# myroslavlisniak/lsm_storage_engine

Hardware: AMD Instinct MI355X
Metric: GiB/s device-resident batched record checksum; % of HBM3E read BW (higher is better)
Workload: dtype u8; 1 GPU; config3: 67108864 mixed-length records per GPU (64 B-64 KiB, Zipf s=1.5, packed, unaligned; 97.0 GiB), device-resident; records_per_gpu=67108864, payload_bytes_per_gpu=104143148313, parallelism=record-sharded x1, no data-path collective, checksum=CRC-32/ISO-HDLC (crc::crc32::checksum_ieee)

## Files before the change

lsm_storage_engine_amd/csrc/lsmck_crc32.hip:

```cpp
#include <hip/hip_runtime.h>
#include <stdint.h>
#ifdef LSMCK_WAVE_DIAG
#include <stdio.h>
#include <stdlib.h>

#include <vector>
#endif

#include "lsmck_device.h"
#include "lsmck_splan.h"

namespace lsmck {

typedef unsigned int u32x4 __attribute__((ext_vector_type(4)));

#define LDS_TABLE_BYTES 131072u
#define LDS_SHIFT_OFF 131072u
#define LDS_SHIFT_BYTES 12288u
#define LDS_COLS_OFF (LDS_SHIFT_OFF + LDS_SHIFT_BYTES)
#define LDS_COLS_BYTES 8192u
#define LDS_KHI_OFF (LDS_COLS_OFF + LDS_COLS_BYTES)
#define LDS_KHI_BYTES 2048u
#define LDS_KLO_OFF (LDS_KHI_OFF + LDS_KHI_BYTES)
#define LDS_KMID_OFF (LDS_KLO_OFF + 2048u)
#define LDS_TINIT_OFF (LDS_KMID_OFF + 512u)
#define LDS_SCRATCH_OFF (LDS_TINIT_OFF + 544u)
#define WAVE_SCRATCH_BYTES 256u
#define LDS_SMAP_OFF LDS_SCRATCH_OFF
#define LDS_SMAP_BYTES 4096u
__device__ __forceinline__ uint32_t gf2_mulmod(uint32_t a, uint32_t b) {
  uint32_t p = 0;
#pragma unroll
  for (int i = 0; i < 32; ++i) {
    uint32_t m = (uint32_t)((int32_t)(a << i) >> 31);
    p ^= b & m;
    b = (b >> 1) ^ (0xEDB88320u & (0u - (b & 1u)));
  }
  return p;
}

__host__ __device__ __forceinline__ uint32_t segs_of(uint32_t len) { return (len >> 7) + ((len & 127u) != 0u); }

typedef __attribute__((address_space(3))) const uint32_t lds_u32_t;
typedef __attribute__((address_space(3))) const u32x4 lds_u32x4_t;
__device__ __forceinline__ uint32_t lds_ld(const unsigned char* smem, uint32_t a) {
  (void)smem;
  return *(lds_u32_t*)(size_t)a;
}
__device__ __forceinline__ u32x4 lds_ld128(uint32_t a) { return *(lds_u32x4_t*)(size_t)a; }

__device__ __forceinline__ void build_lds_tables(unsigned char* smem, const CrcParams& P) {
  const uint32_t* __restrict__ master = P.master;
  uint32_t* s32 = (uint32_t*)smem;
  for (uint32_t i = threadIdx.x; i < LDS_TABLE_BYTES / 4; i += blockDim.x) {
    uint32_t t = ((i >> 14) << 1) | ((i >> 5) & 1u);
    uint32_t e = (i >> 6) & 255u;
    s32[i] = master[t * 256u + e];
  }
  for (uint32_t i = threadIdx.x; i < LDS_SHIFT_BYTES / 4; i += blockDim.x) s32[LDS_SHIFT_OFF / 4 + i] = master[1024u + i];
  for (uint32_t i = threadIdx.x; i < LDS_KHI_BYTES / 4; i += blockDim.x) s32[LDS_KHI_OFF / 4 + i] = P.khi[i];
  for (uint32_t i = threadIdx.x; i < 512u; i += blockDim.x) s32[LDS_KLO_OFF / 4 + i] = P.kseg[i];
  for (uint32_t i = threadIdx.x; i < 128u; i += blockDim.x) s32[LDS_KMID_OFF / 4 + i] = P.kseg[512u * i];
  for (uint32_t i = threadIdx.x; i < 130u; i += blockDim.x) s32[LDS_TINIT_OFF / 4 + i] = P.tinit[i];
}

template <int M>
__device__ __forceinline__ uint32_t shift_bytes32(const unsigned char* smem, uint32_t s) {
  constexpr uint32_t base = LDS_SHIFT_OFF + (M - 1) * 4096u;
  return lds_ld(smem, base + ((s & 0xFFu) << 2)) ^ lds_ld(smem, base + 1024u + (((s >> 8) & 0xFFu) << 2)) ^
         lds_ld(smem, base + 2048u + (((s >> 16) & 0xFFu) << 2)) ^ lds_ld(smem, base + 3072u + ((s >> 24) << 2));
}


__device__ __forceinline__ uint32_t crc_word(const unsigned char* smem, uint32_t s, uint32_t w, uint32_t lo,
                                             uint32_t hi) {
  uint32_t x = s ^ w;
  uint32_t a0 = __builtin_amdgcn_perm(x, hi, 0x0c020400u);
  uint32_t a1 = __builtin_amdgcn_perm(x, hi, 0x0c020500u);
  uint32_t a2 = __builtin_amdgcn_perm(x, lo, 0x0c0c0600u);
  uint32_t a3 = __builtin_amdgcn_perm(x, lo, 0x0c0c0700u);
  return lds_ld(smem, a0 + 128u) ^ lds_ld(smem, a1) ^ lds_ld(smem, a2 + 128u) ^ lds_ld(smem, a3);
}

__device__ __forceinline__ uint32_t crc_step_x(const unsigned char* smem, uint32_t x, uint32_t w_next, uint32_t lo,
                                               uint32_t hi) {
  uint32_t a0 = __builtin_amdgcn_perm(x, hi, 0x0c020400u);
  uint32_t a1 = __builtin_amdgcn_perm(x, hi, 0x0c020500u);
  uint32_t a2 = __builtin_amdgcn_perm(x, lo, 0x0c0c0600u);
  uint32_t a3 = __builtin_amdgcn_perm(x, lo, 0x0c0c0700u);
  const uint32_t l2 = lds_ld(smem, a2 + 128u), l3 = lds_ld(smem, a3);
  const uint32_t t = __builtin_amdgcn_bitop3_b32(l2, l3, w_next, 0x96);
  return __builtin_amdgcn_bitop3_b32(lds_ld(smem, a0 + 128u), lds_ld(smem, a1), t, 0x96);
}

__device__ __forceinline__ void crc_step_x2(uint32_t& c0, uint32_t& c1, uint32_t x0, uint32_t n0, uint32_t x1,
                                            uint32_t n1, uint32_t lo, uint32_t hi) {
  const uint32_t a00 = __builtin_amdgcn_perm(x0, hi, 0x0c020400u), a01 = __builtin_amdgcn_perm(x0, hi, 0x0c020500u);
  const uint32_t a02 = __builtin_amdgcn_perm(x0, lo, 0x0c0c0600u), a03 = __builtin_amdgcn_perm(x0, lo, 0x0c0c0700u);
  const uint32_t a10 = __builtin_amdgcn_perm(x1, hi, 0x0c020400u), a11 = __builtin_amdgcn_perm(x1, hi, 0x0c020500u);
  const uint32_t a12 = __builtin_amdgcn_perm(x1, lo, 0x0c0c0600u), a13 = __builtin_amdgcn_perm(x1, lo, 0x0c0c0700u);
  const uint32_t l02 = lds_ld(nullptr, a02 + 128u), l03 = lds_ld(nullptr, a03);
  const uint32_t l00 = lds_ld(nullptr, a00 + 128u), l01 = lds_ld(nullptr, a01);
  const uint32_t l12 = lds_ld(nullptr, a12 + 128u), l13 = lds_ld(nullptr, a13);
  const uint32_t l10 = lds_ld(nullptr, a10 + 128u), l11 = lds_ld(nullptr, a11);
  c0 = __builtin_amdgcn_bitop3_b32(l00, l01, __builtin_amdgcn_bitop3_b32(l02, l03, n0, 0x96), 0x96);
  c1 = __builtin_amdgcn_bitop3_b32(l10, l11, __builtin_amdgcn_bitop3_b32(l12, l13, n1, 0x96), 0x96);
}

__device__ __forceinline__ uint32_t ld32(const unsigned char* p) { return *(const uint32_t*)p; }
__device__ __forceinline__ u32x4 ld128(const unsigned char* p) { return *(const u32x4*)p; }

template <typename T>
__device__ __forceinline__ void keep_live(const T& x) {
  asm volatile("" ::"v"(x));
}

struct SegInfo {
  uint32_t rec;
  uint32_t q;
  uint32_t k;
  uint64_t rec_off;
  uint32_t rec_len;
  bool valid;
};

struct SegLoad {
  uint32_t d[33];
  uint32_t rec, k;
  uint32_t fl;
};
#define FL_SH(f) ((f) & 3u)
#define FL_BST(f) (((f) >> 2) & 0xFFu)
#define FL_VALID 0x400u
#define FL_FIRST 0x800u
#define FL_M(f) (((f) >> 12) & 0x3Fu)

template <bool FAST, int ABLATE = 0>
__device__ __forceinline__ void seg_issue(const CrcParams& P, const SegInfo& si, SegLoad& L) {
  const uint64_t E = si.rec_off + si.rec_len - 128ull * si.k;
  const uint32_t seglen = (si.q == 0) ? si.rec_len - 128u * si.k : 128u;
  const uint32_t lead = 128u - seglen;
  L.rec = si.rec;
  L.k = si.k;
  const uint32_t flv = (si.valid ? FL_VALID : 0u) | (si.q == 0 ? FL_FIRST : 0u);
  L.fl = flv;
  const unsigned char* s0 = P.base + (E - 128);
  if (FAST) {
#pragma unroll
    for (int g = 0; g < 8; ++g) {
      u32x4 v = ld128(s0 + 16 * g);
      L.d[4 * g + 0] = v.x;
      L.d[4 * g + 1] = v.y;
      L.d[4 * g + 2] = v.z;
      L.d[4 * g + 3] = v.w;
    }
    keep_live(s0);
    L.d[32] = 0;
    return;
  }
  const uint32_t sh = (uint32_t)((uintptr_t)s0 & 3);
  const unsigned char* p = s0 - sh;
  const uint32_t bstart = sh + lead;
  const bool empty = lead >= 128u;
  const uintptr_t pa = (uintptr_t)p;
  const uintptr_t pg = (pa + bstart) & ~(uintptr_t)4095;
  const bool cross = !empty & (pg > pa);
  const uint32_t m = cross ? (uint32_t)(pg - pa) >> 2 : 0u;
  L.fl = flv | sh | (bstart << 2) | (m << 12);
  const unsigned char* w = empty ? (const unsigned char*)P.zero : p + 4u * m;
#pragma unroll
  for (int g = 0; g < 8; ++g) {
    u32x4 v = ld128(w + 16 * g);
    L.d[4 * g + 0] = v.x;
    L.d[4 * g + 1] = v.y;
    L.d[4 * g + 2] = v.z;
    L.d[4 * g + 3] = v.w;
  }
  L.d[32] = ld32(w + ((sh != 0u && m == 0u) ? 128 : 124));
  keep_live(w);
}

template <bool FAST, int CHAINS, int ABLATE = 0, bool PERCOL = false, bool RAW = false>
// ... 653 lines not shown
                                  lds_ld(nullptr, (((v >> 10) & 0x3C0u) | bA) + 4096u), 0x96);
  u = __builtin_amdgcn_bitop3_b32(u, lds_ld(nullptr, (((v >> 14) & 0x3C0u) | bA) + 5120u),
                                  lds_ld(nullptr, (((v >> 18) & 0x3C0u) | bA) + 6144u), 0x96);
  u ^= lds_ld(nullptr, (((v >> 22) & 0x3C0u) | bA) + 7168u);
  uint32_t y = __builtin_amdgcn_bitop3_b32(lds_ld(nullptr, ((u << 2) & 0x3Cu) | bB),
                                           lds_ld(nullptr, (((u >> 2) & 0x3Cu) | bB) + 256u),
                                           lds_ld(nullptr, (((u >> 6) & 0x3Cu) | bB) + 512u), 0x96);
  y = __builtin_amdgcn_bitop3_b32(y, lds_ld(nullptr, (((u >> 10) & 0x3Cu) | bB) + 768u),
                                  lds_ld(nullptr, (((u >> 14) & 0x3Cu) | bB) + 1024u), 0x96);
  y = __builtin_amdgcn_bitop3_b32(y, lds_ld(nullptr, (((u >> 18) & 0x3Cu) | bB) + 1280u),
                                  lds_ld(nullptr, (((u >> 22) & 0x3Cu) | bB) + 1536u), 0x96);
  return y ^ lds_ld(nullptr, (((u >> 26) & 0x3Cu) | bB) + 1792u);
}

__device__ __forceinline__ uint32_t stream_capture(const unsigned char* smem, uint32_t cx, uint32_t u, uint32_t t,
                                                   uint32_t lo) {
  const uint32_t b0 = t == 1u ? lo : (t == 2u ? lo + 128u : (lo | 0x10000u));
  const uint32_t b1 = t == 2u ? lo : lo + 128u;
  const uint32_t l0 = lds_ld(smem, __builtin_amdgcn_perm(cx, b0, 0x0c020400u));
  const uint32_t l1 = lds_ld(smem, __builtin_amdgcn_perm(cx, b1, 0x0c020500u));
  const uint32_t l2 = lds_ld(smem, __builtin_amdgcn_perm(cx, lo, 0x0c020600u));
  return ((cx ^ u) >> (t << 3)) ^ (t >= 1u ? l0 : 0u) ^ (t >= 2u ? l1 : 0u) ^ (t >= 3u ? l2 : 0u);
}


__device__ __forceinline__ void stream_cut(const CrcParams& P, uint32_t w, uint32_t S, uint32_t W) {
  const uint64_t n = P.nrec;
  if (w == S) {
    P.scuts[w] = n;
    return;
  }
  const uint64_t o0 = P.off[0], dend = P.off[n - 1] + P.len[n - 1];
  const uint64_t target = o0 + (uint64_t)((double)(dend - o0) * splan::fraction(w, S, W));
  uint64_t a = 0, b = n;
  while (a < b) {
    const uint64_t m = (a + b) >> 1;
    if (P.off[m] < target) a = m + 1; else b = m;
  }
  P.scuts[w] = a;
}

template <bool VEC>
__global__ __launch_bounds__(256) void stream_check(CrcParams P, uint32_t S, uint32_t W) {
  const uint64_t n = P.nrec;
  const uint32_t gt = blockIdx.x * 256u + threadIdx.x;
  if (gt == 0u) P.sflag[1] = 0u;
  if (gt <= S) stream_cut(P, gt, S, W);
  const uint64_t i0 = (uint64_t)gt * 4u;
  uint64_t o[5];
  uint32_t l[5];
  if (VEC && i0 + 4u <= n) {
    const u32x4 a = *(const u32x4*)(P.off + i0), b = *(const u32x4*)(P.off + i0 + 2u);
    const u32x4 c = *(const u32x4*)(P.len + i0);
    o[0] = ((uint64_t)a.y << 32) | a.x;
    o[1] = ((uint64_t)a.w << 32) | a.z;
    o[2] = ((uint64_t)b.y << 32) | b.x;
    o[3] = ((uint64_t)b.w << 32) | b.z;
    l[0] = c.x; l[1] = c.y; l[2] = c.z; l[3] = c.w;
  } else {
#pragma unroll
    for (int j = 0; j < 4; ++j) {
      const uint64_t i = i0 + j < n ? i0 + j : n - 1u;
      o[j] = P.off[i];
      l[j] = P.len[i];
    }
  }
  o[4] = ((uint64_t)(uint32_t)__shfl_down((int)(uint32_t)(o[0] >> 32), 1) << 32) | (uint32_t)__shfl_down((int)(uint32_t)o[0], 1);
  l[4] = (uint32_t)__shfl_down((int)l[0], 1);
  if ((threadIdx.x & 63u) == 63u && i0 + 4u < n) {
    o[4] = P.off[i0 + 4u];
    l[4] = P.len[i0 + 4u];
  }
  bool bad = i0 == 0 && n > 0 && l[0] == 0u;
#pragma unroll
  for (int j = 0; j < 4; ++j) {
    const uint64_t e = o[j] + l[j];
    bad = bad || (i0 + j + 1u < n && (o[j + 1] < e || o[j + 1] - e > STREAM_MAX_GAP || (l[j + 1] == 0u && o[j + 1] != e)));
  }
  if (bad) *P.sflag = 0u;
}

__global__ __launch_bounds__(256) void stream_cuts(CrcParams P, uint32_t S, uint32_t W) {
  const uint32_t w = blockIdx.x * blockDim.x + threadIdx.x;
  if (w == 0u) P.sflag[1] = 0u;
  if (w > S || !*P.sflag) return;
  stream_cut(P, w, S, W);
}

template <int ABLATE>
__device__ __forceinline__ void stream_issue(const CrcParams& P, int64_t tb, uintptr_t end4, uint32_t lane,
                                             uint32_t (&u)[32], uint32_t c0 = 0u) {
  const uintptr_t t0 = (uintptr_t)P.base + (uintptr_t)tb;
  const uint64_t span = end4 - t0;
  const __amdgpu_buffer_rsrc_t r = __builtin_amdgcn_make_buffer_rsrc(
      const_cast<unsigned char*>(P.base + tb), (short)0, (int)(span < 0x7FFFFFFFull ? span : 0x7FFFFFFFull), 0x00020000);
  const uint32_t vo = lane >= c0 ? lane * 128u : 0x80000000u;
  if (ABLATE == 2 || ABLATE == 4 || ABLATE == 10 || ABLATE == 11) {
#pragma unroll
    for (int j = 0; j < 32; ++j) u[j] = (uint32_t)tb * 0x9E3779B1u + lane + j;
    return;
  }
#pragma unroll
  for (int g = 0; g < 8; ++g) {
    auto v = __builtin_amdgcn_raw_buffer_load_b128(r, vo + 16u * g, 0, 0);
    u[4 * g + 0] = v[0];
    u[4 * g + 1] = v[1];
    u[4 * g + 2] = v[2];
    u[4 * g + 3] = v[3];
  }
  keep_live(vo);
}

__device__ __forceinline__ uint32_t stream_short(const CrcParams& P, const unsigned char* smem, int64_t tb, int32_t re,
                                                 uint32_t L, bool on, uint32_t jmin, uint32_t lo, uint32_t hi) {
  const __amdgpu_buffer_rsrc_t r = __builtin_amdgcn_make_buffer_rsrc(
      const_cast<unsigned char*>(P.base + (tb - 256)), (short)0, 8192 + 256, 0x00020000);
  const uint32_t e = (uint32_t)(re + 256);
  const uint32_t s = e - L;
  const uint32_t w0 = e - 64u;
  const uint32_t sh = (uint32_t)(((uintptr_t)P.base + (uintptr_t)(tb - 256) + w0) & 3u);
  const uint32_t p4 = w0 - sh;
  uint32_t d[17];
#pragma unroll
  for (int i = 0; i < 17; ++i) {
    const uint32_t a = p4 + 4u * i;
    const bool hit = on && a + 4u > s && a < e;
    d[i] = __builtin_amdgcn_raw_buffer_load_b32(r, hit ? a : 0x80000000u, 0, 0);
  }
  const uint32_t lead = 64u - L;
  uint32_t c = 0;
#pragma unroll
  for (int j = 0; j < 16; ++j) {
    if ((uint32_t)j < jmin) continue;
    uint32_t w = __builtin_amdgcn_alignbyte(d[j + 1], d[j], sh);
    const uint32_t b = 4u * j;
    w = (b + 4u <= lead) ? 0u : (b >= lead ? w : w & (0xFFFFFFFFu << ((lead - b) << 3)));
    c = crc_word(smem, c, w, lo, hi);
  }
  return ~(c ^ lds_ld(smem, LDS_TINIT_OFF + (L << 2)));
}

__device__ __forceinline__ uint32_t horner(uint32_t v, uint32_t d) {
#ifdef LSMCK_HORNER_COLS
  return walk_mulcol(v, d);
#else
  return nib_mul<LDS_NIBA_OFF, LDS_NIBB_OFF>(v, d);
#endif
}

__device__ __forceinline__ uint32_t finish_mul(uint32_t v, uint32_t m) { return stream_mulcol(v, LDS_XMC_OFF(m)); }

#ifdef LSMCK_WAVE_DIAG
#define LSMCK_WAVE_DIAG_MAX 8192u
__device__ uint64_t g_wave_diag[LSMCK_WAVE_DIAG_MAX][4];
#define WAVE_DIAG(...) __VA_ARGS__
#else
#define WAVE_DIAG(...)
#endif

template <int ABLATE = 0>
__global__ __launch_bounds__(1024) void crc32_stream_kernel(CrcParams P) {
  if (!*P.sflag) return;
  WAVE_DIAG(const uint64_t diag_t0 = wall_clock64(); uint32_t diag_ev = 0; uint32_t diag_no = 0;)
  WAVE_DIAG(auto diag_out = [&] {
    const uint32_t w = (blockIdx.x * blockDim.x + threadIdx.x) >> 6;
    if ((threadIdx.x & 63u) == 0u && w < LSMCK_WAVE_DIAG_MAX) {
      g_wave_diag[w][0] = diag_t0;
      g_wave_diag[w][1] = wall_clock64();
      g_wave_diag[w][2] = ((uint64_t)diag_ev << 32) | diag_no;
      g_wave_diag[w][3] = (uint64_t)__builtin_amdgcn_s_getreg((31 << 11) | 4) |
                          ((uint64_t)__builtin_amdgcn_s_getreg((31 << 11) | 20) << 32);
    }
  };)
  extern __shared__ __attribute__((aligned(16))) unsigned char smem[];
  build_lds_tables(smem, P);
  __syncthreads();
#ifdef LSMCK_HORNER_COLS
  build_walk_cols(P);
#else
  build_nib<LDS_NIBA_OFF, LDS_NIBB_OFF>([&](uint32_t e) { return P.kseg[e]; });
#endif
  if (threadIdx.x >= 128u && threadIdx.x < 192u) {
    const uint32_t f = threadIdx.x - 128u;
    uint32_t K = 0x80000000u;
    for (uint32_t i = 0; i < f; ++i) K = (K >> 8) ^ lds_ld(smem, 256u * (K & 0xFFu));
    const uint32_t base = LDS_XMC_OFF(f);
    for (uint32_t i = 0; i < 32u; ++i) {
      *(__attribute__((address_space(3))) uint32_t*)(size_t)(base + 4u * i) = K;
      K = (K >> 1) ^ (0xEDB88320u & (0u - (K & 1u)));
    }
  }
  const uint32_t lane = threadIdx.x & 63u;
  const uint32_t smap = LDS_SMAP_OFF + (threadIdx.x >> 6) * 256u;
  *(__attribute__((address_space(3))) uint32_t*)(size_t)(smap + 4u * lane) = 0u;
  __syncthreads();
  const uint32_t lo = (lane & 31u) * 4u, hi = lo | 0x10000u;
  const uint32_t wave = __builtin_amdgcn_readfirstlane((blockIdx.x * blockDim.x + threadIdx.x) >> 6);
  const uint64_t n = P.nrec;
  const int64_t a0 = (int64_t)((((uintptr_t)P.base + P.off[0]) & ~(uintptr_t)127) - (uintptr_t)P.base);
  typedef __attribute__((address_space(4))) const CrcParams kargs_t;
  kargs_t* ka = (kargs_t*)__builtin_amdgcn_kernarg_segment_ptr();
  for (uint32_t slice = wave;;) {
  asm volatile("" : "+s"(ka));
  const uint32_t nslice = ka->nslice, nwaves = ka->nwaves;
  if (slice >= nslice) break;
  auto uni64 = [](uint64_t v) -> uint64_t {
    return ((uint64_t)(uint32_t)__builtin_amdgcn_readfirstlane((int)(uint32_t)(v >> 32)) << 32) |
           (uint32_t)__builtin_amdgcn_readfirstlane((int)(uint32_t)v);
  };
  const uint64_t r_lo = uni64(ka->scuts[slice]), r_hi = uni64(ka->scuts[slice + 1]);
  if (nslice > nwaves) {
    uint32_t tk = 0;
    if (lane == 0u) tk = atomicAdd(ka->sflag + 1, 1u);
    slice = nwaves + (uint32_t)__builtin_amdgcn_readfirstlane((int)tk);
  } else {
    slice = nslice;
  }
  if (r_lo >= r_hi) continue;
  const uint64_t o_lo = uni64(P.off[r_lo]), e_hi = uni64(P.off[r_hi - 1] + P.len[r_hi - 1]);
  const uint64_t t_first = (uint64_t)((int64_t)o_lo - a0) >> 13;
  const uint64_t t_last = (uint64_t)((int64_t)e_hi - a0) >> 13;
  const uint32_t c_first = (uint32_t)((uint64_t)((int64_t)o_lo - a0) >> 7) & 63u;
  const uintptr_t end4 = ((uintptr_t)P.base + e_hi + 3u) & ~(uintptr_t)3;
  const uint64_t ntile = t_last >= t_first ? t_last - t_first + 1u : 0u;
  auto tbase = [&](uint64_t t) -> int64_t { return a0 + (int64_t)(t << 13); };

  uint64_t Wo;
  uint32_t Wl;
  auto win_load = [&](uint64_t b) {
    const uint64_t i = b + lane;
    const uint64_t ic = i < n ? i : n - 1u;
    Wo = P.off[ic];
    Wl = P.len[ic];
  };
  uint64_t bt = r_lo;
  uint32_t carry = 0;
  win_load(bt);
  uint32_t qv = 0;
  uint64_t qb = r_lo & ~63ull;
  uint32_t qs = (uint32_t)(r_lo & 63u), qf = qs;
  auto qstore = [&](uint32_t v, bool on, uint32_t* out) {
    const __amdgpu_buffer_rsrc_t r =
        __builtin_amdgcn_make_buffer_rsrc((void*)(out + qb), (short)0, 256, 0x00020000);
    if (on && (ABLATE != 6 || v == 0x9E3779B1u)) __builtin_amdgcn_raw_buffer_store_b32(v, r, lane << 2, 0, 0);
  };
  auto qpush = [&](uint32_t v, uint32_t cnt) {
    const uint32_t src = (lane - qf) & 63u;
    const uint32_t val = (uint32_t)__builtin_amdgcn_ds_bpermute((int)(src << 2), (int)v);
    const uint32_t end = qf + cnt;
    qv = (lane >= qf && lane < end) ? val : qv;
    if (end >= 64u) {
      qstore(qv, lane >= qs, P.out);
      qb += 64u;
      qs = 0u;
      qf = end - 64u;
      qv = lane < qf ? val : qv;
    } else {
      qf = end;
    }
  };

  auto bulk = [&](const uint32_t (&U)[32]) {
    if constexpr (ABLATE == 11 || ABLATE == 12) {
      uint32_t y0 = U[0] ^ (lane == 0u ? carry : 0u), y1 = U[8], y2 = U[16], y3 = U[24];
#pragma unroll
      for (int k = 0; k < 8; ++k) {
        y0 = crc_step_x(smem, y0, k + 1 < 8 ? U[k + 1] : 0u, lo, hi);
        y1 = crc_step_x(smem, y1, k + 1 < 8 ? U[9 + k] : 0u, lo, hi);
        y2 = crc_step_x(smem, y2, k + 1 < 8 ? U[17 + k] : 0u, lo, hi);
        y3 = crc_step_x(smem, y3, k + 1 < 8 ? U[25 + k] : 0u, lo, hi);
      }
      uint32_t dy = 63u - lane;
      asm volatile("" : "+v"(dy));
      const uint32_t XY = wave_prefix_xor(horner(shift_bytes32<2>(smem, y0 ^ y1) ^ y2 ^ y3, dy));
      carry = (uint32_t)__builtin_amdgcn_readlane((int)XY, 63);
      return;
    }
    uint32_t z0 = U[0] ^ (lane == 0u ? carry : 0u), z1 = U[16];
#pragma unroll
    for (int k = 0; k < 16; ++k) {
      z0 = crc_step_x(smem, z0, k + 1 < 16 ? U[k + 1] : 0u, lo, hi);
      z1 = crc_step_x(smem, z1, k + 1 < 16 ? U[17 + k] : 0u, lo, hi);
    }
    uint32_t dz = 63u - lane;
    asm volatile("" : "+v"(dz));
    const uint32_t XZ = wave_prefix_xor(horner(shift_bytes32<2>(smem, z0) ^ z1, dz));
    carry = (uint32_t)__builtin_amdgcn_readlane((int)XZ, 63);
  };

  auto process = [&](const uint32_t (&U)[32], uint64_t t, auto&& issue_next) {
    const int64_t tb = tbase(t);
    if constexpr (ABLATE == 9 || ABLATE == 10 || ABLATE == 11) {
      issue_next();
      __builtin_amdgcn_sched_barrier(0);
      bulk(U);
      return;
    }
    bool zf = false;
    if constexpr (ABLATE == 0 || ABLATE >= 6) {
      const uint32_t so_lo = (uint32_t)__builtin_amdgcn_readfirstlane((int)(uint32_t)Wo);
      const uint32_t so_hi = (uint32_t)__builtin_amdgcn_readfirstlane((int)(uint32_t)(Wo >> 32));
      const uint32_t sl = (uint32_t)__builtin_amdgcn_readfirstlane((int)Wl);
      const int64_t s0 = (int64_t)(((uint64_t)so_hi << 32) | so_lo) - tb;
      zf = bt >= r_hi || (s0 + (int64_t)sl >= 8192 && (s0 < 0 || sl < STREAM_LONG));
    }
    uint32_t Kw = 0;
    bool shorts = false;
    uint64_t wb = bt;
    uint32_t nwin = 0;
    uint32_t cntw = 0;
    int32_t re = 8191, rs = 8191;
    bool lng = false, sin = false;
    const uint64_t bt0 = bt;
    bool z = zf;
    if (!zf) {
      for (;;) {
        const int64_t e64 = (int64_t)(Wo + Wl) - tb, s64 = (int64_t)Wo - tb;
        const bool inr = wb + lane < r_hi;
        const bool ends = inr && e64 < 8192;
        cntw = (uint32_t)__builtin_popcountll(__ballot(ends));
        lng = Wl >= STREAM_LONG;
        sin = inr && s64 >= 0 && s64 < 8192;
        re = (int32_t)(ends ? e64 : 8191);
        rs = (int32_t)(s64 < -128 ? -128 : (s64 > 8191 ? 8191 : s64));
        const bool ev_e = ends && lng, ev_s = sin && lng;
        typedef __attribute__((address_space(3))) unsigned char lds_u8w_t;
        if (ev_e) *(lds_u8w_t*)(size_t)(smap + 4u * ((uint32_t)re >> 7) + (((uint32_t)re >> 5) & 2u)) = (unsigned char)((re & 63) + 1);
        if (ev_s) *(lds_u8w_t*)(size_t)(smap + 4u * ((uint32_t)rs >> 7) + (((uint32_t)rs >> 5) & 2u) + 1u) = (unsigned char)((rs & 63) + 1);
        Kw |= wave_or_u32((ev_e ? 1u << (((uint32_t)re & 127u) >> 2) : 0u) | (ev_s ? 1u << (((uint32_t)rs & 127u) >> 2) : 0u));
        shorts = shorts || __any(ends && !lng);
        if (cntw < 64u) break;
        wb += 64u;
        ++nwin;
        win_load(wb);
      }
      bt = wb + cntw;
      z = nwin == 0u && cntw == 0u && !__builtin_amdgcn_readfirstlane((int)(sin && lng));
      const uint32_t src = lane + cntw;
      const int sp = (int)((src & 63u) << 2);
      const uint32_t wlo = (uint32_t)__builtin_amdgcn_ds_bpermute(sp, (int)(uint32_t)Wo);
      const uint32_t whi = (uint32_t)__builtin_amdgcn_ds_bpermute(sp, (int)(uint32_t)(Wo >> 32));
      const uint32_t wl = (uint32_t)__builtin_amdgcn_ds_bpermute(sp, (int)Wl);
      Wo = ((uint64_t)whi << 32) | wlo;
      Wl = wl;
      if (src >= 64u) {
        const uint64_t i2 = bt + lane;
        const uint64_t ic = i2 < n ? i2 : n - 1u;
        Wo = P.off[ic];
        Wl = P.len[ic];
      }
    }
    __builtin_amdgcn_s_setprio(3);
    issue_next();
    __builtin_amdgcn_sched_barrier(0);
    __builtin_amdgcn_s_setprio(0);
    if constexpr (ABLATE == 0 || ABLATE >= 4) {
      if (z || ABLATE == 4 || ABLATE == 5 || ABLATE == 12) {
        WAVE_DIAG(++diag_no;)
        bulk(U);
        return;
      }
    }
    __builtin_amdgcn_s_setprio(1);
    WAVE_DIAG(++diag_ev;)
    typedef __attribute__((address_space(3))) uint32_t lds_u32w_t;
    uint32_t ev = *(lds_u32w_t*)(size_t)(smap + 4u * lane);
    if (ev) *(lds_u32w_t*)(size_t)(smap + 4u * lane) = 0u;
    const uint64_t M1 = __ballot((ev & 0x00FF00FFu) != 0u);
    const uint64_t Ms = __ballot((ev & 0xFF00FF00u) != 0u);
    const bool ke0 = __any((ev & 0xFFu) != 0u), ke1 = __any((ev & 0xFF0000u) != 0u);
    if (ABLATE == 3) {
      uint32_t x = 0;
#pragma unroll
      for (int k = 0; k < 32; ++k) x ^= U[k];
      if (x == 0x9E3779B1u) P.out[0] = x ^ ev;
      __builtin_amdgcn_s_setprio(0);
      return;
    }
    uint32_t c0 = U[0] ^ (lane == 0u ? carry : 0u), c1 = U[16], x0 = 0u, x1 = 0u, ub0 = 0u, ub1 = 0u;
    const uint32_t Km = ABLATE == 8 ? 0u : Kw;
#pragma unroll
    for (int k = 0; k < 16; ++k) {
      const uint32_t w0 = k + 1 < 16 ? U[k + 1] : 0u, w1 = k + 1 < 16 ? U[17 + k] : 0u;
      uint32_t i0 = c0, i1 = c1, n0 = w0, n1 = w1;
      if (Km & (1u << k)) {
        uint32_t e = ev;
        asm volatile("" : "+v"(e));
        const uint32_t e3 = e + 0x03030303u;
        if (((e3 >> 2) & 0x3Fu) == (uint32_t)(k + 1)) {
          x0 = c0;
          ub0 = U[k];
          asm volatile("" : "+v"(x0), "+v"(ub0));
        }
        if (((e3 >> 10) & 0x3Fu) == (uint32_t)(k + 1)) {
          const uint32_t mlo0 = (1u << ((e3 >> 5) & 0x18u)) - 1u;
          i0 = ~(U[k] | mlo0);
          n0 = w0 ^ mlo0;
          asm volatile("" : "+v"(i0), "+v"(n0));
        }
      }
      if (Km & (1u << (16 + k))) {
        uint32_t e = ev;
        asm volatile("" : "+v"(e));
        const uint32_t e3 = e + 0x03030303u;
        if (((e3 >> 18) & 0x3Fu) == (uint32_t)(k + 1)) {
          x1 = c1;
          ub1 = U[16 + k];
          asm volatile("" : "+v"(x1), "+v"(ub1));
        }
        if ((e3 >> 26) == (uint32_t)(k + 1)) {
          const uint32_t mlo1 = (1u << ((e3 >> 21) & 0x18u)) - 1u;
          i1 = ~(U[16 + k] | mlo1);
          n1 = w1 ^ mlo1;
          asm volatile("" : "+v"(i1), "+v"(n1));
        }
      }
      crc_step_x2(c0, c1, i0, n0, i1, n1, lo, hi);
    }
    const uint32_t cap0 = ke0 ? stream_capture(smem, x0, ub0, ((ev & 0xFFu) - 1u) & 3u, lo) : 0u;
    const uint32_t cap1 = ke1 ? stream_capture(smem, x1, ub1, (((ev >> 16) & 0xFFu) - 1u) & 3u, lo) : 0u;
    const uint32_t R0 = c0;
    const uint32_t T = (ev >> 24) ? c1 : (shift_bytes32<2>(smem, c0) ^ c1);
    uint32_t l1 = lane + 1u;
    asm volatile("" : "+v"(l1));
    const uint64_t above = lane == 63u ? 0ull : (M1 >> l1) << l1;
    const uint32_t cn = above ? (uint32_t)__builtin_ctzll(above) : 64u;
    const uint32_t X = wave_prefix_xor(horner(T, cn - 1u - lane));
    auto finish = [&](uint32_t cnt, int32_t re_, int32_t rs_, bool lng_, bool sin_) -> uint32_t {
      const uint32_t c = (uint32_t)re_ >> 7, j = (uint32_t)re_ & 127u;
      const uint32_t Ye = (uint32_t)__builtin_amdgcn_ds_bpermute((int)(((c - 1u) & 63u) << 2), (int)X);
      const uint32_t cs = (uint32_t)rs_ >> 7;
      const uint32_t Ys = (uint32_t)__builtin_amdgcn_ds_bpermute((int)(((cs - 1u) & 63u) << 2), (int)X);
      const uint32_t H = (c ? Ye : 0u) ^ ((sin_ && cs) ? Ys : 0u);
      const int sc = (int)(c << 2);
      const uint32_t R0c = (uint32_t)__builtin_amdgcn_ds_bpermute(sc, (int)R0);
      const uint32_t A0c = (uint32_t)__builtin_amdgcn_ds_bpermute(sc, (int)cap0);
      const uint32_t A1c = (uint32_t)__builtin_amdgcn_ds_bpermute(sc, (int)cap1);
      const bool in = lane < cnt;
      uint32_t fv = 0u;
      if (in && lng_ && ABLATE != 7) {
        const bool h = j >= 64u;
        const uint32_t Pv = h ? (shift_bytes32<2>(smem, H) ^ R0c) : H;
        fv = ~(finish_mul(Pv, j & 63u) ^ (h ? A1c : A0c));
      }
      return fv;
    };
    auto finish_short = [&](uint32_t fv, uint32_t cnt, int32_t re_, int32_t rs_, bool lng_) -> uint32_t {
      const bool sh = lane < cnt && !lng_;
      const uint32_t L = sh ? (uint32_t)(re_ - rs_) : 0u;
      const int need = sh ? (int)((L + 3u) >> 2) : 0;
      const uint32_t jmin = 16u - (uint32_t)__builtin_amdgcn_readlane(wave_prefix_max(need), 63);
      const uint32_t v = stream_short(P, smem, tb, re_, L, sh, jmin, lo, hi);
      return sh ? v : fv;
    };
    for (uint32_t k = 0; k < nwin; ++k) {
      const uint64_t i = bt0 + 64u * k + lane;
      const uint64_t o = P.off[i];
      const uint32_t l = P.len[i];
      const int64_t s64 = (int64_t)o - tb;
      const int32_t kre = (int32_t)((int64_t)(o + l) - tb);
      const int32_t krs = (int32_t)(s64 < -128 ? -128 : s64);
      const bool klng = l >= STREAM_LONG;
      uint32_t fv = finish(64u, kre, krs, klng, s64 >= 0);
      if (__any(!klng)) fv = finish_short(fv, 64u, kre, krs, klng);
      qpush(fv, 64u);
    }
    if (cntw) {
      uint32_t fv = finish(cntw, re, rs, lng, sin);
      if (shorts && __any(lane < cntw && !lng)) fv = finish_short(fv, cntw, re, rs, lng);
      qpush(fv, cntw);
    }
    const uint32_t X63 = (uint32_t)__builtin_amdgcn_readlane((int)X, 63);
    const uint32_t cl = Ms ? 63u - (uint32_t)__builtin_clzll(Ms) : 0u;
    carry = X63 ^ (cl ? (uint32_t)__builtin_amdgcn_readlane((int)X, (int)(cl - 1u)) : 0u);
    __builtin_amdgcn_s_setprio(0);
  };

  auto tcl = [&](uint64_t x) -> int64_t { return tbase(x < ntile ? t_first + x : t_last); };
  auto none = [] {};
  uint32_t U0[32], U1[32];
  uint64_t i = 0;
  stream_issue<ABLATE>(P, tcl(0), end4, lane, U0, c_first);
  for (; i + 2 <= ntile; i += 2) {
    process(U0, t_first + i, [&] { stream_issue<ABLATE>(P, tcl(i + 1), end4, lane, U1); });
    process(U1, t_first + i + 1, [&] { stream_issue<ABLATE>(P, tcl(i + 2), end4, lane, U0); });
  }
  if (i < ntile) process(U0, t_first + i, none);
  if ((ABLATE == 4 || ABLATE == 5 || ABLATE == 7 || ABLATE >= 9) && carry == 0x9E3779B1u) P.out[0] = carry;
  if (ABLATE == 3) continue;
  asm volatile("" : "+s"(ka));
  qstore(qv, lane >= qs && lane < qf, ka->out);
  }
  WAVE_DIAG(diag_out();)
}
}

using namespace lsmck;


template <bool FAST, bool PERCOL>
static int launch_fixed(const CrcParams* P, int ncu, hipStream_t st) {
  size_t lds = LDS_SCRATCH_OFF;
  hipError_t e = hipFuncSetAttribute((const void*)crc32_fixed_kernel<FAST, 2, 0, PERCOL>,
                                     hipFuncAttributeMaxDynamicSharedMemorySize, (int)lds);
  if (e != hipSuccess) return -(int)e;
  hipLaunchKernelGGL((crc32_fixed_kernel<FAST, 2, 0, PERCOL>), dim3(ncu), dim3(1024), lds, st, *P);
  e = hipGetLastError();
  return e == hipSuccess ? 0 : -(int)e;
}

template <int ABLATE>
static int launch_wring(const CrcParams* P, int ncu, hipStream_t st) {
  size_t lds = LDS_SCRATCH_OFF;
  hipError_t e = hipFuncSetAttribute((const void*)crc32_wring_kernel<2, ABLATE>,
                                     hipFuncAttributeMaxDynamicSharedMemorySize, (int)lds);
  if (e != hipSuccess) return -(int)e;
  hipLaunchKernelGGL((crc32_wring_kernel<2, ABLATE>), dim3(ncu), dim3(1024), lds, st, *P);
  e = hipGetLastError();
  return e == hipSuccess ? 0 : -(int)e;
}

extern "C" int lsmk_launch_crc32_fixed(const CrcParams* P, int ncu, int variant, hipStream_t st) {
  const bool fast = ((uintptr_t)P->base % 4 == 0) && (P->stride % 4 == 0) && (P->flen % 128 == 0);
  const uint32_t nsegr = segs_of(P->flen);
  const bool percol = (64u % nsegr) == 0;
  const bool buf_ok = (uint64_t)P->stride * 65u + P->flen < (1ull << 31);
  const int ablate = (variant >> 8) & 0xF;
  if (fast && percol && buf_ok) return ablate == 3 ? launch_wring<3>(P, ncu, st) : launch_wring<0>(P, ncu, st);
  if (fast && percol) return launch_fixed<true, true>(P, ncu, st);
  if (fast) return launch_fixed<true, false>(P, ncu, st);
  return launch_fixed<false, false>(P, ncu, st);
}

extern "C" uint32_t lsmk_stream_slices_max(int ncu) { return splan::slices_max(ncu); }

extern "C" int lsmk_ab_ablations() {
#ifdef LSMCK_AB_ABLATIONS
  return 1;
#else
  return 0;
#endif
}

extern "C" int lsmk_launch_crc32_stream(const CrcParams* P, int ncu, int variant, int trusted, hipStream_t st) {
  const uint64_t n = P->nrec;
  if (n == 0) return 0;
  hipError_t e = hipMemsetAsync(P->sflag, 1, 4, st);
  if (e != hipSuccess) return -(int)e;
  const uint32_t W = splan::slices(ncu, n), NW = splan::waves(ncu);
  if (!trusted) {
    const bool vec = ((uintptr_t)P->off % 16u == 0) && ((uintptr_t)P->len % 16u == 0);
    const uint64_t nb = std::max<uint64_t>((n + 1023) / 1024, (W + 1u + 255u) / 256u);
    const dim3 g((unsigned)nb);
    if (vec) hipLaunchKernelGGL(stream_check<true>, g, dim3(256), 0, st, *P, W, NW);
    else hipLaunchKernelGGL(stream_check<false>, g, dim3(256), 0, st, *P, W, NW);
  } else {
    hipLaunchKernelGGL(stream_cuts, dim3((W + 1u + 255u) / 256u), dim3(256), 0, st, *P, W, NW);
  }
  const int ablate = (variant >> 8) & 0xF;
#ifdef LSMCK_AB_ABLATIONS
  const void* fn = ablate == 11 ? (const void*)crc32_stream_kernel<11>
                 : ablate == 12 ? (const void*)crc32_stream_kernel<12>
                 : ablate == 9 ? (const void*)crc32_stream_kernel<9>
                 : ablate == 10 ? (const void*)crc32_stream_kernel<10>
                 : ablate == 4 ? (const void*)crc32_stream_kernel<4>
                 : ablate == 5 ? (const void*)crc32_stream_kernel<5>
                 : ablate == 6 ? (const void*)crc32_stream_kernel<6>
                 : ablate == 7 ? (const void*)crc32_stream_kernel<7>
                 : ablate == 8 ? (const void*)crc32_stream_kernel<8>
                 : ablate == 3 ? (const void*)crc32_stream_kernel<3>
                 : ablate == 2 ? (const void*)crc32_stream_kernel<2> : (const void*)crc32_stream_kernel<0>;
#else
  const void* fn = ablate == 3 ? (const void*)crc32_stream_kernel<3> : (const void*)crc32_stream_kernel<0>;
#endif
  const size_t lds = LDS_SCRATCH_OFF + LDS_SMAP_BYTES;
  e = hipFuncSetAttribute(fn, hipFuncAttributeMaxDynamicSharedMemorySize, (int)lds);
  if (e != hipSuccess) return -(int)e;
  CrcParams Q = *P;
  Q.nslice = W;
  Q.nwaves = NW;
  void* args[] = {(void*)&Q};
  e = hipLaunchKernel(fn, dim3(ncu), dim3(1024), args, lds, st);
  if (e != hipSuccess) return -(int)e;
  e = hipGetLastError();
#ifdef LSMCK_WAVE_DIAG
  if (const char* path = getenv("LSMCK_WAVE_DIAG_OUT")) {
    const uint32_t nw = std::min<uint32_t>((uint32_t)ncu * 16u, LSMCK_WAVE_DIAG_MAX);
    std::vector<uint64_t> h(4u * (nw + 1u));
    h[0] = 0x4741494445564157ull;
    h[1] = nw;
    h[2] = n;
    h[3] = 0;
    if (hipStreamSynchronize(st) == hipSuccess &&
        hipMemcpyFromSymbol(h.data() + 4, HIP_SYMBOL(g_wave_diag), 32u * nw) == hipSuccess) {
      if (FILE* f = fopen(path, "ab")) {
        fwrite(h.data(), 8, h.size(), f);
        fclose(f);
      }
    }
  }
#endif
  return e == hipSuccess ? 0 : -(int)e;
}

extern "C" uint64_t lsmk_walk_sb_count(uint64_t n) { return (n + WALK_SB - 1) / WALK_SB; }

extern "C" int lsmk_launch_crc32_walk(const CrcParams* P, uint64_t* sb_prefix, int ncu, int variant,
                                      hipStream_t st) {
  const uint64_t n = P->nrec;
  if (n == 0) return 0;
  const uint64_t nsb = lsmk_walk_sb_count(n);
  const uint64_t nblk = std::min<uint64_t>((nsb + 15) / 16, (uint64_t)ncu * 2u);
  hipLaunchKernelGGL(walk_phase1, dim3((unsigned)nblk), dim3(1024), 0, st, P->len, n, sb_prefix,
                     (const uint32_t*)P->sflag);
  hipLaunchKernelGGL(scan_phase2, dim3(1), dim3(1024), 0, st, sb_prefix, (uint32_t)nsb, P->total_segs,
                     (const uint32_t*)P->sflag);
  CrcParams Q = *P;
  Q.sb_prefix = sb_prefix;
  const int ablate = (variant >> 8) & 0xF;
  const void* fn = ablate == 3 ? (const void*)crc32_walk_kernel<2, 3> : (const void*)crc32_walk_kernel<2>;
  size_t lds = LDS_SCRATCH_OFF;
  hipError_t e = hipFuncSetAttribute(fn, hipFuncAttributeMaxDynamicSharedMemorySize, (int)lds);
  if (e != hipSuccess) return -(int)e;
  void* args[] = {(void*)&Q};
  e = hipLaunchKernel(fn, dim3(ncu), dim3(1024), args, lds, st);
  if (e != hipSuccess) return -(int)e;
  e = hipGetLastError();
  return e == hipSuccess ? 0 : -(int)e;
}

namespace lsmck {
__global__ __launch_bounds__(256) void crc32_compare_kernel(const uint32_t* __restrict__ crc,
                                                             const uint32_t* __restrict__ expected, uint64_t n,
                                                             unsigned long long* __restrict__ n_bad,
                                                             unsigned long long* __restrict__ first_bad) {
  uint64_t i = (uint64_t)blockIdx.x * blockDim.x + threadIdx.x;
  uint64_t stride = (uint64_t)gridDim.x * blockDim.x;
  unsigned long long bad = 0, first = ~0ull;
  for (; i < n; i += stride) {
    if (crc[i] != expected[i]) {
      ++bad;
      if (i < first) first = i;
    }
  }
  if (bad) {
    atomicAdd(n_bad, bad);
    atomicMin(first_bad, first);
  }
}
}

extern "C" int lsmk_launch_crc32_compare(const uint32_t* crc, const uint32_t* expected, uint64_t n,
                                          unsigned long long* n_bad, unsigned long long* first_bad, hipStream_t st) {
  if (n == 0) return 0;
  uint64_t blocks = (n + 255) / 256;
  if (blocks > 8192) blocks = 8192;
  hipLaunchKernelGGL(crc32_compare_kernel, dim3((unsigned)blocks), dim3(256), 0, st, crc, expected, n, n_bad,
                     first_bad);
  hipError_t e = hipGetLastError();
  return e == hipSuccess ? 0 : -(int)e;
}
```

lsm_storage_engine_amd/csrc/lsmck_splan.h:

```cpp
#ifndef LSMCK_SPLAN_H
#define LSMCK_SPLAN_H
#include <stdint.h>

#if defined(__HIPCC__)
#define LSMCK_SPLAN_HD __host__ __device__
#else
#define LSMCK_SPLAN_HD
#endif

#ifndef STREAM_SLICES
#define STREAM_SLICES 16u
#endif
#ifndef STREAM_PLAN_F0
#define STREAM_PLAN_F0 72u
#endif
#ifndef STREAM_PLAN_R
#define STREAM_PLAN_R 50u
#endif
#ifndef STREAM_PLAN_FLOOR
#define STREAM_PLAN_FLOOR 3u
#endif

static_assert(STREAM_SLICES >= 1u && STREAM_SLICES <= 64u, "slices per wave");
static_assert(STREAM_PLAN_F0 < 100u, "the first region's share is a percentage under 100");
static_assert(STREAM_PLAN_R >= 1u && STREAM_PLAN_R <= 100u, "a ticket group is no larger than the one before");
static_assert(STREAM_PLAN_FLOOR <= 20u, "the floor is a shift of the first group's 2^20");

namespace lsmck {
namespace splan {

LSMCK_SPLAN_HD inline uint32_t waves(int ncu) { return (uint32_t)ncu * 16u; }
LSMCK_SPLAN_HD inline uint32_t slices_max(int ncu) { return waves(ncu) * STREAM_SLICES; }

LSMCK_SPLAN_HD inline uint32_t slices(int ncu, uint64_t n) {
  const uint64_t w = waves(ncu), hi = w * STREAM_SLICES, by_rec = n / 64u;
  const uint64_t s = by_rec > w ? by_rec : w;
  return (uint32_t)(s < hi ? s : hi);
}

LSMCK_SPLAN_HD inline uint64_t group_weight(uint32_t g) {
  const uint64_t lo = (1u << 20) >> STREAM_PLAN_FLOOR;
  uint64_t w = 1u << 20;
  for (uint32_t i = 0; i < g && w > lo; ++i) w = w * STREAM_PLAN_R / 100u;
  return w > lo ? w : lo;
}

LSMCK_SPLAN_HD inline uint64_t ticket_prefix(uint32_t t, uint32_t W) {
  uint64_t p = 0;
  uint32_t g = 0;
  for (; t >= W; t -= W, ++g) p += (uint64_t)W * group_weight(g);
  return p + (uint64_t)t * group_weight(g);
}

LSMCK_SPLAN_HD inline double fraction(uint32_t s, uint32_t S, uint32_t W) {
  if (s >= S) return 1.0;
  if (S <= W) return (double)s / (double)S;
  const uint64_t tk = ticket_prefix(S - W, W);
  uint64_t first = (STREAM_PLAN_F0 * tk + (100u - STREAM_PLAN_F0) * W - 1u) / ((100u - STREAM_PLAN_F0) * W);
  if (first < (1u << 20)) first = 1u << 20;
  const uint64_t total = first * W + tk;
  const uint64_t p = s <= W ? first * s : first * W + ticket_prefix(s - W, W);
  return (double)p / (double)total;
}

}
}
#endif
```

Before: 5573 GiB/s.

## Pace lagging waves in a workgroup via LDS progress counters and priority boost

Each wave publishes its tile progress to a small LDS array. Every few tile pairs it sums the progress of the 16 waves in its workgroup with DPP and raises its own s_setprio by one level when it lags the group average by more than a set number of tiles. This is meant to even out completion times across waves of the first slice so the tail shrinks. The slice plan is retuned alongside it: fewer slices per wave, a larger first-region share and a higher floor. The added LDS traffic and the periodic reduction cost a little per tile pair.

```diff
diff --git a/lsm_storage_engine_amd/csrc/lsmck_crc32.hip b/lsm_storage_engine_amd/csrc/lsmck_crc32.hip
--- a/lsm_storage_engine_amd/csrc/lsmck_crc32.hip
+++ b/lsm_storage_engine_amd/csrc/lsmck_crc32.hip
@@ -28,6 +28,14 @@
 #define WAVE_SCRATCH_BYTES 256u
 #define LDS_SMAP_OFF LDS_SCRATCH_OFF
 #define LDS_SMAP_BYTES 4096u
+#define LDS_PROG_OFF (LDS_SMAP_OFF + LDS_SMAP_BYTES)
+#define LDS_PROG_BYTES 64u
+#define LDS_STREAM_BYTES (LDS_PROG_OFF + LDS_PROG_BYTES)
+static_assert(LDS_STREAM_BYTES <= 160u * 1024u, "the stream kernel's LDS stays within a CU's 160 KiB");
+static_assert(LDS_PROG_OFF >= LDS_SMAP_OFF + 16u * 256u, "prog lies behind the last wave's event map");
+static_assert(LDS_PROG_OFF >= LDS_SCRATCH_OFF && LDS_SCRATCH_OFF >= LDS_TINIT_OFF + 544u,
+              "prog lies behind every table (all of them end at LDS_SCRATCH_OFF)");
+static_assert(LDS_PROG_OFF % 4u == 0u, "prog holds dwords");
 __device__ __forceinline__ uint32_t gf2_mulmod(uint32_t a, uint32_t b) {
   uint32_t p = 0;
 #pragma unroll
@@ -987,16 +995,38 @@
 
 #ifdef LSMCK_WAVE_DIAG
 #define LSMCK_WAVE_DIAG_MAX 8192u
-__device__ uint64_t g_wave_diag[LSMCK_WAVE_DIAG_MAX][4];
+#define LSMCK_WAVE_DIAG_WORDS 5u
+__device__ uint64_t g_wave_diag[LSMCK_WAVE_DIAG_MAX][LSMCK_WAVE_DIAG_WORDS];
 #define WAVE_DIAG(...) __VA_ARGS__
 #else
 #define WAVE_DIAG(...)
 #endif
 
+#ifndef STREAM_PACE
+#define STREAM_PACE 1
+#endif
+#ifndef STREAM_PACE_PERIOD
+#define STREAM_PACE_PERIOD 16u
+#endif
+#ifndef STREAM_PACE_LAG
+#define STREAM_PACE_LAG 8u
+#endif
+static_assert(STREAM_PACE_PERIOD >= 2u && (STREAM_PACE_PERIOD & (STREAM_PACE_PERIOD - 1u)) == 0u,
+              "the look falls on a trip of the two-tile loop: an even power of two");
+#if STREAM_PACE
+#define STREAM_SETPRIO(X)                          \
+  do {                                             \
+    if (pb) __builtin_amdgcn_s_setprio((X) + 1);   \
+    else __builtin_amdgcn_s_setprio(X);            \
+  } while (0)
+#else
+#define STREAM_SETPRIO(X) __builtin_amdgcn_s_setprio(X)
+#endif
+
 template <int ABLATE = 0>
 __global__ __launch_bounds__(1024) void crc32_stream_kernel(CrcParams P) {
   if (!*P.sflag) return;
-  WAVE_DIAG(const uint64_t diag_t0 = wall_clock64(); uint32_t diag_ev = 0; uint32_t diag_no = 0;)
+  WAVE_DIAG(const uint64_t diag_t0 = wall_clock64(); uint32_t diag_ev = 0; uint32_t diag_no = 0; uint64_t diag_fs = 0;)
   WAVE_DIAG(auto diag_out = [&] {
     const uint32_t w = (blockIdx.x * blockDim.x + threadIdx.x) >> 6;
     if ((threadIdx.x & 63u) == 0u && w < LSMCK_WAVE_DIAG_MAX) {
@@ -1005,6 +1035,7 @@
       g_wave_diag[w][2] = ((uint64_t)diag_ev << 32) | diag_no;
       g_wave_diag[w][3] = (uint64_t)__builtin_amdgcn_s_getreg((31 << 11) | 4) |
                           ((uint64_t)__builtin_amdgcn_s_getreg((31 << 11) | 20) << 32);
+      g_wave_diag[w][4] = diag_fs;
     }
   };)
   extern __shared__ __attribute__((aligned(16))) unsigned char smem[];
@@ -1028,6 +1059,16 @@
   const uint32_t lane = threadIdx.x & 63u;
   const uint32_t smap = LDS_SMAP_OFF + (threadIdx.x >> 6) * 256u;
   *(__attribute__((address_space(3))) uint32_t*)(size_t)(smap + 4u * lane) = 0u;
+#if STREAM_PACE
+  typedef __attribute__((address_space(3))) uint32_t lds_prog_t;
+  auto prog_put = [&](uint32_t v) {
+    uint32_t a = smap;
+    asm volatile("" : "+v"(a));
+    if (lane == 0u) *(lds_prog_t*)(size_t)(LDS_PROG_OFF + ((a - LDS_SMAP_OFF) >> 6)) = v;
+  };
+  prog_put(0u);
+  uint32_t pb = 0u;
+#endif
   __syncthreads();
   const uint32_t lo = (lane & 31u) * 4u, hi = lo | 0x10000u;
   const uint32_t wave = __builtin_amdgcn_readfirstlane((blockIdx.x * blockDim.x + threadIdx.x) >> 6);
@@ -1039,6 +1080,10 @@
   asm volatile("" : "+s"(ka));
   const uint32_t nslice = ka->nslice, nwaves = ka->nwaves;
   if (slice >= nslice) break;
+#if STREAM_PACE
+  const bool pace = __builtin_amdgcn_readfirstlane((int)(slice < nwaves && (nslice > nwaves || STREAM_SLICES == 1u))) != 0;
+  pb = 0u;
+#endif
   auto uni64 = [](uint64_t v) -> uint64_t {
     return ((uint64_t)(uint32_t)__builtin_amdgcn_readfirstlane((int)(uint32_t)(v >> 32)) << 32) |
            (uint32_t)__builtin_amdgcn_readfirstlane((int)(uint32_t)v);
@@ -1188,7 +1233,7 @@
     __builtin_amdgcn_s_setprio(3);
     issue_next();
     __builtin_amdgcn_sched_barrier(0);
-    __builtin_amdgcn_s_setprio(0);
+    STREAM_SETPRIO(0);
     if constexpr (ABLATE == 0 || ABLATE >= 4) {
       if (z || ABLATE == 4 || ABLATE == 5 || ABLATE == 12) {
         WAVE_DIAG(++diag_no;)
@@ -1196,7 +1241,7 @@
         return;
       }
     }
-    __builtin_amdgcn_s_setprio(1);
+    STREAM_SETPRIO(1);
     WAVE_DIAG(++diag_ev;)
     typedef __attribute__((address_space(3))) uint32_t lds_u32w_t;
     uint32_t ev = *(lds_u32w_t*)(size_t)(smap + 4u * lane);
@@ -1209,7 +1254,7 @@
 #pragma unroll
       for (int k = 0; k < 32; ++k) x ^= U[k];
       if (x == 0x9E3779B1u) P.out[0] = x ^ ev;
-      __builtin_amdgcn_s_setprio(0);
+      STREAM_SETPRIO(0);
       return;
     }
     uint32_t c0 = U[0] ^ (lane == 0u ? carry : 0u), c1 = U[16], x0 = 0u, x1 = 0u, ub0 = 0u, ub1 = 0u;
@@ -1308,7 +1353,7 @@
     const uint32_t X63 = (uint32_t)__builtin_amdgcn_readlane((int)X, 63);
     const uint32_t cl = Ms ? 63u - (uint32_t)__builtin_clzll(Ms) : 0u;
     carry = X63 ^ (cl ? (uint32_t)__builtin_amdgcn_readlane((int)X, (int)(cl - 1u)) : 0u);
-    __builtin_amdgcn_s_setprio(0);
+    STREAM_SETPRIO(0);
   };
 
   auto tcl = [&](uint64_t x) -> int64_t { return tbase(x < ntile ? t_first + x : t_last); };
@@ -1317,11 +1362,36 @@
   uint64_t i = 0;
   stream_issue<ABLATE>(P, tcl(0), end4, lane, U0, c_first);
   for (; i + 2 <= ntile; i += 2) {
+#if STREAM_PACE
+    if (pace) {
+      prog_put((uint32_t)i);
+      if (((uint32_t)i & (STREAM_PACE_PERIOD - 1u)) == 0u) {
+        uint32_t pl = lane;
+        asm volatile("" : "+v"(pl));
+        uint32_t s = *(lds_prog_t*)(size_t)(LDS_PROG_OFF + 4u * (pl & 15u));
+        s += (uint32_t)__builtin_amdgcn_update_dpp(0, (int)s, 0x128, 0xF, 0xF, false);
+        s += (uint32_t)__builtin_amdgcn_update_dpp(0, (int)s, 0x124, 0xF, 0xF, false);
+        s += (uint32_t)__builtin_amdgcn_update_dpp(0, (int)s, 0x122, 0xF, 0xF, false);
+        s += (uint32_t)__builtin_amdgcn_update_dpp(0, (int)s, 0x121, 0xF, 0xF, false);
+        const uint32_t sum = (uint32_t)__builtin_amdgcn_readfirstlane((int)s);
+        const uint32_t own = (uint32_t)__builtin_amdgcn_readfirstlane((int)(uint32_t)i);
+        pb = 16u * (own + STREAM_PACE_LAG) < sum ? 1u : 0u;
+      }
+    }
+#endif
     process(U0, t_first + i, [&] { stream_issue<ABLATE>(P, tcl(i + 1), end4, lane, U1); });
     process(U1, t_first + i + 1, [&] { stream_issue<ABLATE>(P, tcl(i + 2), end4, lane, U0); });
   }
   if (i < ntile) process(U0, t_first + i, none);
+#if STREAM_PACE
+  if (pace) {
+    prog_put((uint32_t)ntile);
+    pb = 0u;
+    __builtin_amdgcn_s_setprio(0);
+  }
+#endif
   if ((ABLATE == 4 || ABLATE == 5 || ABLATE == 7 || ABLATE >= 9) && carry == 0x9E3779B1u) P.out[0] = carry;
+  WAVE_DIAG(if (!diag_fs) diag_fs = wall_clock64();)
   if (ABLATE == 3) continue;
   asm volatile("" : "+s"(ka));
   qstore(qv, lane >= qs && lane < qf, ka->out);
@@ -1408,7 +1478,7 @@
 #else
   const void* fn = ablate == 3 ? (const void*)crc32_stream_kernel<3> : (const void*)crc32_stream_kernel<0>;
 #endif
-  const size_t lds = LDS_SCRATCH_OFF + LDS_SMAP_BYTES;
+  const size_t lds = LDS_STREAM_BYTES;
   e = hipFuncSetAttribute(fn, hipFuncAttributeMaxDynamicSharedMemorySize, (int)lds);
   if (e != hipSuccess) return -(int)e;
   CrcParams Q = *P;
@@ -1421,13 +1491,13 @@
 #ifdef LSMCK_WAVE_DIAG
   if (const char* path = getenv("LSMCK_WAVE_DIAG_OUT")) {
     const uint32_t nw = std::min<uint32_t>((uint32_t)ncu * 16u, LSMCK_WAVE_DIAG_MAX);
-    std::vector<uint64_t> h(4u * (nw + 1u));
+    std::vector<uint64_t> h(4u + LSMCK_WAVE_DIAG_WORDS * nw);
     h[0] = 0x4741494445564157ull;
     h[1] = nw;
     h[2] = n;
-    h[3] = 0;
+    h[3] = LSMCK_WAVE_DIAG_WORDS;
     if (hipStreamSynchronize(st) == hipSuccess &&
-        hipMemcpyFromSymbol(h.data() + 4, HIP_SYMBOL(g_wave_diag), 32u * nw) == hipSuccess) {
+        hipMemcpyFromSymbol(h.data() + 4, HIP_SYMBOL(g_wave_diag), 8u * LSMCK_WAVE_DIAG_WORDS * nw) == hipSuccess) {
       if (FILE* f = fopen(path, "ab")) {
         fwrite(h.data(), 8, h.size(), f);
         fclose(f);
diff --git a/lsm_storage_engine_amd/csrc/lsmck_splan.h b/lsm_storage_engine_amd/csrc/lsmck_splan.h
--- a/lsm_storage_engine_amd/csrc/lsmck_splan.h
+++ b/lsm_storage_engine_amd/csrc/lsmck_splan.h
@@ -9,16 +9,16 @@
 #endif
 
 #ifndef STREAM_SLICES
-#define STREAM_SLICES 16u
+#define STREAM_SLICES 8u
 #endif
 #ifndef STREAM_PLAN_F0
-#define STREAM_PLAN_F0 72u
+#define STREAM_PLAN_F0 88u
 #endif
 #ifndef STREAM_PLAN_R
 #define STREAM_PLAN_R 50u
 #endif
 #ifndef STREAM_PLAN_FLOOR
-#define STREAM_PLAN_FLOOR 3u
+#define STREAM_PLAN_FLOOR 2u
 #endif
 
 static_assert(STREAM_SLICES >= 1u && STREAM_SLICES <= 64u, "slices per wave");
```

Result: no change. 5599 GiB/s (median of 6 runs) (+0.5%).
